# tmbdev/clstm

Hardware: AMD Instinct MI355X
Metric: text-line images/sec (fwd+bwd+CTC), 100-unit BiLSTM H=48 T~200 (higher is better)
Workload: dtype f32 (operand-exact split): forward, recurrences, CTC, decode in f32 arithmetic; the backward weight-gradient / softmax-backward products take their f32 operands split EXACTLY into three bf16 terms each (x1 + x2 + x3 = x) and sum the six bf16-MFMA products of weight >= 2^-16 in f32 -- what is dropped

## Files before the change

clstm_amd/csrc/dbgopt.h:

```cpp
#pragma once
#include <cstdlib>
#include <cstring>
#include <map>
#include <stdexcept>
#include <string>

namespace clstm {
struct DbgOptDef { const char* name; int dflt; };
inline constexpr DbgOptDef DBG_OPTS[] = {
    {"gemm_stag", 2},
    {"bwd_c32", 1},
    {"rec_x3", 1},
    {"pack_tiles", 1},
    {"fuse_wx", 1},
    {"gemm_b16mc", 1},
    {"dw_x3", 1},
    {"gemm_x3", 1},
    {"split_terms", 3},
    {"fwd_mfma", 1},
    {"bwd_mfma", 1},
    {"bwd_mfma_fused", 1},
    {"ctc_float", 0},
    {"peer_two_phase", 1},
};
inline const DbgOptDef* dbg_opt_def(const char* name) {
  for (const DbgOptDef& o : DBG_OPTS)
    if (strcmp(o.name, name) == 0) return &o;
  return nullptr;
}
inline std::map<std::string, int>& dbg_opts() {
  static std::map<std::string, int> m = [] {
    std::map<std::string, int> r;
    const char* e = getenv("CLSTM_DEBUG");
    if (e) {
      std::string s(e);
      size_t i = 0;
      while (i < s.size()) {
        size_t j = s.find(',', i);
        if (j == std::string::npos) j = s.size();
        const std::string kv = s.substr(i, j - i);
        const size_t eq = kv.find('=');
        if (!kv.empty()) {
          const std::string name = kv.substr(0, eq);
          if (eq == std::string::npos || !dbg_opt_def(name.c_str()))
            throw std::runtime_error("CLSTM_DEBUG: unknown option '" + name + "' (clstm_amd/csrc/dbgopt.h lists them as name=value)");
          r[name] = atoi(kv.c_str() + eq + 1);
        }
        i = j + 1;
      }
    }
    return r;
  }();
  return m;
}
inline int dbg_opt(const char* name) {
  const DbgOptDef* d = dbg_opt_def(name);
  if (!d) throw std::logic_error(std::string("internal: option '") + name + "' is not in DBG_OPTS");
  const auto& m = dbg_opts();
  const auto it = m.find(name);
  return it == m.end() ? d->dflt : it->second;
}
}
```

clstm_amd/csrc/gemm_dw.h:

```cpp
#pragma once
#include <type_traits>
#include "gemm_bf16.h"

namespace clstm {

struct DwSlab {
  int tile_begin, ntiles;
  int need_it;
  int dir;
  int out_z;
  int pad[3];
};

struct GemmDwArgs {
  const float* S; long long sdir; int lds; long long s_elems;
  const float* D; int M; int no4; long long d_elems;
  const int* ktab;
  int ntiles_max;
  const DwSlab* slabs;
  int nslabs;
  const int* prog;
  const int* line_off;
  int bs, prog_base, ndir;
  float* partial;
  int R, Cn;
  unsigned gx, gy;
  int* timeouts;
  int* minprog;
  int tcap;
  int* done;
  int done_target;
  long long* trace;
  int trace_base;
  const float* xS; int xlds; long long xs_elems;
  const float* xD; int xM; long long xd_elems;
  const int* xtab; const DwSlab* xslabs; int xnslabs;
  float* xpartial; int xR, xCn; unsigned xgx, xgy;
  int x3;
  int terms;
};

constexpr int DW_PF = 3;
constexpr int DW_STAB_MAX = 256;
constexpr int dw_img_floats(int nt) { return nt <= 2 ? 8192 : 2 * 2 * nt * 64 * 32 / 2; }
constexpr int dw_smem_floats(int nt) { return dw_img_floats(nt) + 2 * DW_STAB_MAX; }
static_assert(8192 >= GEMM_BT * GEMM_LDO, "epilogue tile");

constexpr int DW_WATCHDOG_POLLS = 1 << 16;

DEVFN void gemm_dw_monitor(const GemmDwArgs& a) {
  if (threadIdx.x >= 64) return;
  const int lane = threadIdx.x & 63;
  int polls = 0;
  for (;;) {
    int all = 0x3fffffff;
    int pv[2][4];
#pragma unroll
    for (int dir = 0; dir < 2; dir++)
#pragma unroll
      for (int j = 0; j < 4; j++) {
        const int b = lane + 64 * j;
        pv[dir][j] = dir < a.ndir && b < a.bs ? load_i32_wt(a.prog + ((size_t)dir * a.bs + b) * PROG_STRIDE) : 0;
      }
    for (int dir = 0; dir < a.ndir; dir++) {
      int m = 0x3fffffff;
      for (int b = lane, j = 0; b < a.bs; b += 64, j++) {
        const int T = a.line_off[b + 1] - a.line_off[b];
        const int p = (j < 4 ? pv[dir][j] : load_i32_wt(a.prog + ((size_t)dir * a.bs + b) * PROG_STRIDE)) - a.prog_base;
        const int v = p >= T ? 0x3fffffff : (p < 0 ? 0 : p);
        m = v < m ? v : m;
      }
      m = -wave_max_i(-m);
      if (lane == 0) store_i32_wt(a.minprog + dir * PROG_STRIDE, a.prog_base + (m > a.tcap ? a.tcap : m));
      all = m < all ? m : all;
    }
    if (all >= 0x3fffffff) break;
    if (++polls > (DW_WATCHDOG_POLLS << 4)) {
      if (lane == 0) {
        atomic_add_i32(a.timeouts, 1);
        for (int dir = 0; dir < a.ndir; dir++) store_i32_wt(a.minprog + dir * PROG_STRIDE, a.prog_base + a.tcap);
      }
      break;
    }
  }
}

DEVFN void gemm_dw_wait(const GemmDwArgs& a, const int dir, const int need_it) {
  const int wave = wave_uniform(threadIdx.x >> 6);
  if (wave == 0) {
    const int need = need_it < a.tcap ? need_it : a.tcap;
    const bool all = a.done && need_it >= a.tcap - 32;
    int polls = 0;
// ... 288 lines not shown
```

clstm_amd/csrc/lstm_bwd_dw.h:

```cpp
#pragma once
#include "gemm_dw.h"
#include "lstm_seq.h"

namespace clstm {

constexpr int DW_FUSED_STAB_ENTRIES = 1024;
static_assert(DW_FUSED_STAB_ENTRIES >= DW_STAB_MAX, "the items' k-tile table fits");

template <int NK4, int KU, int NT>
__global__ __launch_bounds__(64 * NK4) CLSTM_TWO_WAVES_PER_SIMD void lstm_bwd_dw_kernel(LstmSeqArgs a, GemmDwArgs g, int nrec) {
  __shared__ __attribute__((aligned(16))) float gsm[dw_img_floats(NT) + 2 * DW_FUSED_STAB_ENTRIES];
  if ((int)blockIdx.x < nrec) {
#ifndef CLSTM_HIP_EMU
    __builtin_amdgcn_s_setprio(3);
#endif
    const long long t0 = g.trace ? wall_clock() : 0;
    const int bl = (int)blockIdx.x % a.bs;
    lstm_bwd_body<NK4, KU>(a, a.order ? a.order[bl] : bl, (int)blockIdx.x / a.bs);
    if (g.done && threadIdx.x == 0) atomic_add_i32(g.done, 1);
    if (g.trace && threadIdx.x == 0) { g.trace[blockIdx.x * 4] = t0; g.trace[blockIdx.x * 4 + 2] = wall_clock(); }
  } else {
    if (threadIdx.x >= 256) return;
    gemm_dw_body<NT>(g, gsm, blockIdx.x - (unsigned)nrec);
  }
}

}
```

clstm_amd/csrc/net.inc:

```
struct Layer {
  int ni, no, nk4, nthreads;
  bool wide = false;
  int kpf = 0, kpb = 0;
  long long nwf = 0, nwb = 0;
  PackDesc pd;
  float *Wt = nullptr, *bias = nullptr, *Rf = nullptr, *Rb = nullptr, *Rwf = nullptr, *Rwb = nullptr;
  float* Wk = nullptr;
  int wk_kp = 0, wk_njp = 0;
  DevBuf<float> dCc;
  DevBuf<unsigned short> Wmf;
  DevBuf<float> mf_scale;
  DevBuf<unsigned> mf_xmax;
  long long mf_epoch = -1;
  DevBuf<unsigned short> Wmfb;
  long long mfb_epoch = -1;
  DevBuf<int> pack_tab;
  DevBuf<int> pack_inv;
  int pack_inv_state = 0;
  unsigned short *Rbf = nullptr, *Rbb = nullptr;
  DevBuf<unsigned short> R2b, D2;
  bool r2b_ready = false;
  DevBuf<unsigned short> Hb, Db;
  DevBuf<float> Rf32;
  long long* moff = nullptr;
// ... 534 lines not shown
    const int mode = dbg_opt("bwd_mfma");
    if (!mode || y.wide || bf16_gemm) return false;
    if (strict_f32 && mode < 2) return false;
    if (!(y.no == 64 || y.no == 100)) return false;
    const double lim = 2147483000.0;
    if ((double)N * ndir * 4 * y.no * 4 >= lim) return false;
    return mode >= 2 || bs >= 640;
#endif
  }
#ifndef CLSTM_HIP_EMU
  template <int NO, int NT>
  LstmMfmaBwdArgs mfma_bwd_args(Layer& y, const LstmSeqArgs& sa, hipStream_t s) {
    using Gm = MfmaBwdGeom<NO, NT>;
    if (y.mfb_epoch != params_epoch) {
      y.Wmfb.reserve((size_t)ndir * Gm::W_HALFS_PER_DIR + 64);
      MfmaBwdPackArgs p{};
      p.v = v; p.ni = y.ni; p.no = y.no; p.ntl = Gm::NTL; p.kb = Gm::KB; p.nt = NT; p.W = y.Wmfb.p;
      for (int d = 0; d < 2; d++) for (int q = 0; q < 4; q++) p.p_off[d][q] = y.pd.p_off[d][q];
      CLSTM_LAUNCH(k_pack_mfma_bwd, dim3(64, (unsigned)ndir), dim3(256), 0, s, p);
      y.mfb_epoch = params_epoch;
    }
    LstmMfmaBwdArgs a{};
    a.W = y.Wmfb.p; a.G = sa.G; a.C = sa.C; a.dH = sa.dH; a.D = sa.D; a.line_off = sa.line_off; a.order = sa.order;
    a.bs = bs; a.ndir = ndir; a.N = N; a.prog_off = sa.prog_off; a.prog_base = sa.prog_base;
    return a;
  }
  template <int NO>
  void launch_mfma_bwd_no(Layer& y, const LstmSeqArgs& sa, hipStream_t s) {
    constexpr int NT = 2;
    using Gr = MfmaBwdRowsGeom<NO, NT>;
    const LstmMfmaBwdArgs a = mfma_bwd_args<NO, NT>(y, sa, s);
    static const bool smem_set = (coop_set_smem(lstm_bwd_mfma_rows_kernel<NO, NT>, (size_t)Gr::SMEM), true);
    (void)smem_set;
    CLSTM_LAUNCH((lstm_bwd_mfma_rows_kernel<NO, NT>), dim3((unsigned)((bs + 15) / 16), (unsigned)ndir), dim3(512), (size_t)Gr::SMEM, s, a);
    g_path_count[PC_MFMA_BWD]++;
  }
  template <int NO>
  bool launch_mfma_bwd_dw_no(Layer& y, const LstmSeqArgs& sa, const GemmDwArgs& g, unsigned ngemm, hipStream_t s) {
    constexpr int NT = 2;
    using Gr = MfmaBwdRowsGeom<NO, NT>;
    const LstmMfmaBwdArgs a = mfma_bwd_args<NO, NT>(y, sa, s);
    const int ngroups = (bs + 15) / 16, nrec = ngroups * ndir;
    static const bool smem_set = (coop_set_smem(lstm_bwd_mfma_dw_kernel<NO, NT, 3>, (size_t)Gr::SMEM), true);
    (void)smem_set;
    CLSTM_LAUNCH((lstm_bwd_mfma_dw_kernel<NO, NT, 3>), dim3((unsigned)nrec + ngemm), dim3(512), (size_t)Gr::SMEM, s, a, g, nrec, ngroups);
    g_path_count[PC_MFMA_BWD]++; g_path_count[PC_MFMA_BWD_DW]++;
    return true;
  }
  bool mfma_bwd_fused_ok(const Layer& y, const GemmDwArgs& g) const {
    const int mode = dbg_opt("bwd_mfma_fused");
    return mfma_bwd_eligible(y) && mode && g.x3 && g.terms >= 3 && (mode >= 2 || bs < 900);
  }
#endif
  void launch_bwd_narrow(Layer& y, const LstmSeqArgs& a, hipStream_t s) {
#ifndef CLSTM_HIP_EMU
    if (mfma_bwd_eligible(y)) {
      if (y.no == 64) launch_mfma_bwd_no<64>(y, a, s);
      else launch_mfma_bwd_no<100>(y, a, s);
      check_launch();
      return;
    }
#endif
    launch_lstm(false, y.nk4, y.pd.ku, a, bs, y.nthreads, s);
  }
  void launch_mfma(Layer& y, bool fwd, hipStream_t s, bool save = true) {
#ifndef CLSTM_HIP_EMU
    if (save) {
      if (y.no == 64) launch_mfma_no<64, 48>(y, fwd, s);
      else if (y.no == 100) launch_mfma_no<100, 48>(y, fwd, s);
      else launch_mfma_no<128, 48>(y, fwd, s);
    } else {
      REQUIRE(mfma_nosave_ok(y), "internal: no no-save instantiation of the batched recurrence for this layer");
      if (y.no == 64) launch_mfma_no<64, 48, false>(y, fwd, s);
      else launch_mfma_no<100, 48, false>(y, fwd, s);
    }
    check_launch();
#else
    (void)y; (void)fwd; (void)s; (void)save;
#endif
  }

  void forward() {
    REQUIRE(N > 0, "set_batch first");
    RoctxRange range_("clstm:forward");
    ensure_training_buffers();
    nosave = false;
    forward_pass(true);
  }
  void forward_pass(bool save) {
    flush_line_off();
    repack();
    hipStream_t s = stream();
    if (forward_family(L[0]) == FwdFamily::Fused) { forward_fused(save); return; }
    for (int l = 0; l < (int)L.size(); l++) {
      Layer& y = L[l];
      const int M = ndir * 4 * y.no;
      const FwdFamily fam = forward_family(y);
      const bool x_from_hbf = bf16_gemm && bf16_rec && l > 0 && L[l - 1].fwd_persistent && L[l - 1].Hbf.p && y.WtbT.p && y.ni == ndir * L[l - 1].no && (y.ni & 1) == 0;
      auto run_wide = [&](LstmWideArgs w, int fx_ngx) {
        timing.begin("lstm_fwd", s);
        const WideRan ran = launch_lstm_wide(true, w, tmax, coop_sync, step_graphs, s, bf16_rec, fx_ngx);
        timing.end(s);
        if (ran == WideRan::Nothing) return false;
        y.fwd_persistent = ran == WideRan::Persistent && bf16_rec;
        y.h_f32_valid = !(y.fwd_persistent && w.skip_h);
        y.sh_valid = !(y.fwd_persistent && w.skip_s);
        if (ran == WideRan::Persistent) g_path_count[PC_FWD_PERSISTENT]++;
// ... 180 lines not shown
    h.pitems = fw_items.p; h.npitems = fw_npitems; h.gflag = fw_flags.p;
    h.W1k = W1k; h.kps = w1k_kps; h.sm_k = sm_ni; h.b1 = v + sm_off; h.Z = Z.p; h.nc = desc.nclasses;
    h.citems = fw_items.p + 4 * fw_npitems; h.ncitems = fw_ncitems;
    h.nanflag = fwd_nanflag(); h.step_no = step_no() + 1;
    h.prog = (const int*)(y.H.p + a.prog_off);
    h.nrec = bs * ndir; h.npb = fw_npitems;
    const unsigned nblk = (unsigned)(h.nrec + h.npb + fw_ncitems);
    if (save) { y.sx_valid = src0_ready; ensure_source_x(0); }
    static const char* trace_path = getenv("CLSTM_FW_TRACE");
    const size_t trace_rows = (size_t)h.nrec + fw_npitems + fw_ncitems;
    if (trace_path) { dw_trace.reserve(trace_rows * 4); HIPCHECK(hipMemsetAsync(dw_trace.p, 0, trace_rows * 4 * sizeof(long long), s)); h.trace = dw_trace.p; }
    timing.begin("lstm_fwd", s);
    REQUIRE(launch_lstm_fwd_fused(y.nk4, y.pd.ku, k, nblk, y.nthreads, s, save), "internal: no fused forward instantiation");
    timing.end(s);
    if (trace_path)
      dump_trace(trace_path, dw_trace.p, trace_rows, s,
                 "# %d recurrence rows (start - end -), %d producer items (start - done chunk), %d consumer items (start ready done ready_iteration); 100 MHz ticks\n",
                 h.nrec, fw_npitems, fw_ncitems);
  }

  bool dw_x3 = dbg_opt("dw_x3") != 0;
  int split_terms = dbg_opt("split_terms");
  bool gemm_x3_on = dbg_opt("gemm_x3") != 0;
  bool strict_f32 = false;
  bool rec_x3() const {
    if (bf16_gemm || bf16_rec || !gemm_x3_on) return false;
    return dbg_opt("rec_x3") != 0;
  }
  int clamp_split(long long want) const { return (int)std::max(1LL, std::min({want, (long long)(N + 63) / 64, 64LL})); }
  int pick_split_mc(int R, int Cn, int nbatch) const {
    const int th = gemm_mc_tile_rows(R);
    const long long tiles = (long long)((R + th - 1) / th) * ((Cn + 255) / 256) * nbatch;
    return clamp_split(device_cu_count() / tiles);
  }
  int pick_split(int R, int Cn, int nbatch = 1, int tile = GEMM_BT) const {
    const long long tiles = (long long)((R + tile - 1) / tile) * ((Cn + tile - 1) / tile) * nbatch;
    const long long target = tile == GEMM_BT ? 640 : 480;
    long long want = (target + tiles - 1) / tiles;
    if (tile == 256) want = device_cu_count() / tiles;
    return clamp_split(want);
  }

  bool overlap_eligible(const Layer& y) const {
    if (!overlap || y.wide || y.no % 16 == 0) return false;
    if (bs > PROG_LINES) return false;
    if ((overlap == 1) && (tmax < 64 || N < 2048)) return false;
    if ((double)y.D.cap * 4.0 >= 2147483000.0) return false;
    return overlap == 2 || y.nthreads >= 256;
  }
  BwdFamily backward_family(const Layer& y) const {
    if (!bf16_gemm && overlap_eligible(y)) return BwdFamily::Overlapped;
    return y.wide ? BwdFamily::Wide : BwdFamily::Narrow;
  }
  static int dw_bf16_rows(const Layer& y, int R, int Cn) { return wide_kp16_bwd(y.no) == 4 * y.no && gemm_bf16_big(R - 1, Cn) ? R - 1 : R; }
  static constexpr int DW_CHUNK = 16, DW_TAIL_PARTS = 4, DW_TAIL_CHUNKS = 2;
  void build_dw_tables() {
    if (dw_key == line_off_h && dw_nslabs > 0) return;
    std::vector<int> cb;
    for (int done = DW_CHUNK; done < tmax; done += DW_CHUNK) cb.push_back(done);
    cb.push_back(tmax);
    const int tiles_per_slab = std::min(DW_STAB_MAX, std::max(8, (int)((N / 16 + 15) / 16)));
    std::vector<std::vector<int>> tab(ndir);
    struct Sl { int tb, nt, need, dir, chunk, part; };
    std::vector<std::vector<Sl>> sl(ndir);
    for (int dir = 0; dir < ndir; dir++) {
      int cs = 0;
      for (size_t c = 0; c < cb.size(); c++) {
        const int ce = cb[c];
        const int t0 = (int)tab[dir].size() / 2;
        for (int b = 0; b < bs; b++) {
          const int off = line_off_h[b], T = line_off_h[b + 1] - off;
          if (T <= cs) continue;
          const int e = std::min(ce, T);
          const int f_lo = dir == 0 ? T - e : cs, f_hi = dir == 0 ? T - cs : e;
          for (int f = f_lo; f < f_hi; f += 16) { tab[dir].push_back(off + f); tab[dir].push_back(std::min(16, f_hi - f)); }
        }
        const int nt = (int)tab[dir].size() / 2 - t0;
        int parts = std::max(1, (nt + tiles_per_slab - 1) / tiles_per_slab);
        if (c + DW_TAIL_CHUNKS >= cb.size()) parts = std::max(parts, std::min(DW_TAIL_PARTS, std::max(1, nt / 2)));
        for (int p = 0; p < parts; p++) {
          const int a0 = t0 + (int)((long long)nt * p / parts), a1 = t0 + (int)((long long)nt * (p + 1) / parts);
          REQUIRE(a1 - a0 <= DW_STAB_MAX, "internal: weight-gradient slab longer than its LDS table");
          sl[dir].push_back(Sl{a0, a1 - a0, ce, dir, (int)c, p});
        }
        cs = ce;
      }
    }
    dw_slabs_per_dir = (int)sl[0].size();
    for (int dir = 1; dir < ndir; dir++) REQUIRE((int)sl[dir].size() == dw_slabs_per_dir, "internal: asymmetric slab lists");
    dw_ntiles_max = 0;
    for (int dir = 0; dir < ndir; dir++) dw_ntiles_max = std::max(dw_ntiles_max, (int)tab[dir].size() / 2);
    std::vector<DwSlab> slabs;
    for (int i = 0; i < dw_slabs_per_dir; i++)
      for (int dir = 0; dir < ndir; dir++) {
        const Sl& x = sl[dir][i];
        slabs.push_back(DwSlab{x.tb, x.nt, x.need, dir, dir * dw_slabs_per_dir + i, {0, 0, 0}});
      }
    dw_nslabs = (int)slabs.size();
    const size_t nk = (size_t)ndir * dw_ntiles_max * 2, nsw = slabs.size() * sizeof(DwSlab) / sizeof(int);
    dw_ktab.reserve(nk + 8);
    dw_slabs.reserve(nsw + 8);
    hipStream_t s = stream();
    int* stage = (int*)ring.acquire((nk + nsw) * sizeof(int));
    for (int dir = 0; dir < ndir; dir++) {
      std::fill(stage + (size_t)dir * dw_ntiles_max * 2, stage + (size_t)(dir + 1) * dw_ntiles_max * 2, 0);
      std::copy(tab[dir].begin(), tab[dir].end(), stage + (size_t)dir * dw_ntiles_max * 2);
    }
    memcpy(stage + nk, slabs.data(), nsw * sizeof(int));
    HIPCHECK(hipMemcpyAsync(dw_ktab.p, stage, nk * sizeof(int), hipMemcpyHostToDevice, s));
    HIPCHECK(hipMemcpyAsync(dw_slabs.p, stage + nk, nsw * sizeof(int), hipMemcpyHostToDevice, s));
    ring.commit(s);
    dw_key = line_off_h;
  }
  void backward_layer_overlapped(Layer& y, LstmSeqArgs a, int R, int Cn) {
    hipStream_t s = stream();
    build_dw_tables();
    const int M = ndir * 4 * y.no;
    const long long prog_off = (long long)y.D.cap - 64 - PROG_WORDS;
    REQUIRE(prog_off >= (long long)N * M, "internal: progress words overlap the deltas");
    prog_base += tmax + 64;
    dw_launches++;
    if (prog_base > (1 << 30)) prog_base = 1024;
    a.prog_off = prog_off;
    a.prog_base = prog_base;
    DevBuf<float>& partial = layer_partial(y);
    partial.reserve((size_t)ndir * dw_slabs_per_dir * R * Cn);
    GemmDwArgs g{};
    g.S = y.S.p; g.sdir = (long long)N * y.lds; g.lds = y.lds; g.s_elems = (long long)N * ndir * y.lds + 3;
    g.D = y.D.p; g.M = M; g.no4 = 4 * y.no; g.d_elems = (long long)N * M + 3;
    g.ktab = dw_ktab.p; g.ntiles_max = dw_ntiles_max; g.slabs = (const DwSlab*)dw_slabs.p; g.nslabs = dw_nslabs;
    g.prog = (const int*)(y.D.p + prog_off); g.line_off = line_off.p; g.bs = bs; g.prog_base = prog_base;
    g.partial = partial.p; g.R = R; g.Cn = Cn;
    g.gx = (unsigned)((Cn + GEMM_BT - 1) / GEMM_BT); g.gy = (unsigned)((R + GEMM_BT - 1) / GEMM_BT);
    g.timeouts = dev_err_words() + 1;
    if (!dw_queue.p) dw_queue.reserve(5 * PROG_STRIDE);
    g.ndir = ndir;
    g.minprog = dw_queue.p + PROG_STRIDE;
    g.tcap = tmax + 32;
    g.done = nullptr; g.done_target = 0;
    g.x3 = dw_x3;
    g.terms = split_terms;
    unsigned nextra = 0;
    if (dwx_active && &y == &L.back()) {
      const int xR = 1 + sm_ni, xCn = desc.nclasses;
      g.xS = y.srow(); g.xlds = y.ldh; g.xs_elems = (long long)N * y.ldh + 3;
      g.xD = Dz.p; g.xM = xCn; g.xd_elems = (long long)N * xCn + 3;
      g.xtab = dwx_tab.p; g.xslabs = (const DwSlab*)(dwx_tab.p + 2 * dwx_entries); g.xnslabs = dwx_nslabs;
      g.xpartial = partial_sm.p; g.xR = xR; g.xCn = xCn;
      g.xgx = (unsigned)((xCn + GEMM_BT - 1) / GEMM_BT); g.xgy = (unsigned)((xR + GEMM_BT - 1) / GEMM_BT);
      nextra = (unsigned)dwx_nslabs * g.xgx * g.xgy;
    }
    static const char* trace_path = getenv("CLSTM_DW_TRACE");
    const size_t trace_rows = (size_t)bs * ndir + (size_t)((dw_nslabs + 7) / 8) * 8 * g.gx * g.gy + 8;
    if (trace_path) { dw_trace.reserve(trace_rows * 4); g.trace = dw_trace.p; g.trace_base = bs * ndir; }
    const unsigned nblk = 1u + nextra + (unsigned)((dw_nslabs + 7) / 8) * 8u * g.gx * g.gy;
#ifndef CLSTM_HIP_EMU
    if (mfma_bwd_fused_ok(y, g)) {
      timing.begin("lstm_bwd", s);
      g.done = nullptr; g.done_target = 0;
      const bool ok = y.no == 64 ? launch_mfma_bwd_dw_no<64>(y, a, g, nblk, s) : launch_mfma_bwd_dw_no<100>(y, a, g, nblk, s);
      timing.end(s);
      check_launch();
      if (ok) return;
    }
    if (y.nthreads >= 256 && !mfma_bwd_eligible(y)) {
      timing.begin("lstm_bwd", s);
      g.done = g.minprog + 2 * PROG_STRIDE;
      dw_done_total += (unsigned)(bs * ndir);
      g.done_target = (int)dw_done_total;
      REQUIRE(launch_lstm_bwd_dw(y.nk4, y.pd.ku, a, g, bs * ndir, nblk, y.nthreads, s), "internal: no fused instantiation");
      timing.end(s);
      if (trace_path)
        dump_trace(trace_path, dw_trace.p, trace_rows, s,
                   "# rows 0..%d: recurrence workgroups (start, -, end); then one row per (slab, tile) item: start ready done need_it; 100 MHz ticks\n", bs * ndir - 1);
      return;
    }
#endif
    timing.begin("lstm_bwd", s);
    launch_bwd_narrow(y, a, s);
    timing.end(s);
    timing.begin("gemm_gates_dw", s);
    if (g.x3 && g.terms >= 3) CLSTM_LAUNCH(gemm_dw_kernel<3>, dim3(nblk), dim3(256), 0, s, g);
    else if (g.x3) CLSTM_LAUNCH(gemm_dw_kernel<2>, dim3(nblk), dim3(256), 0, s, g);
    else CLSTM_LAUNCH(gemm_dw_kernel<0>, dim3(nblk), dim3(256), 0, s, g);
    timing.end(s);
    check_launch();
  }

  void build_dwx_table() {
    if (dwx_N == N) return;
    hipStream_t s = stream();
    dwx_entries = (int)((N + 15) / 16);
    const int eps = std::min(DW_STAB_MAX, std::max(32, (dwx_entries + 63) / 64));
    dwx_nslabs = (dwx_entries + eps - 1) / eps;
    const size_t nsw = (size_t)dwx_nslabs * sizeof(DwSlab) / sizeof(int);
    dwx_tab.reserve((size_t)2 * dwx_entries + nsw + 8);
    int* stage = (int*)ring.acquire(((size_t)2 * dwx_entries + nsw) * sizeof(int));
    for (int e = 0; e < dwx_entries; e++) { stage[2 * e] = 16 * e; stage[2 * e + 1] = (int)std::min<long long>(16, N - 16LL * e); }
    DwSlab* sl = (DwSlab*)(stage + 2 * dwx_entries);
    for (int i = 0; i < dwx_nslabs; i++) sl[i] = DwSlab{eps * i, std::min(eps, dwx_entries - eps * i), 0, 0, i, {0, 0, 0}};
    for (int i = 0; i < dwx_nslabs; i++) REQUIRE(sl[i].ntiles <= DW_STAB_MAX, "internal: weight-gradient slab longer than its LDS table");
    HIPCHECK(hipMemcpyAsync(dwx_tab.p, stage, ((size_t)2 * dwx_entries + nsw) * sizeof(int), hipMemcpyHostToDevice, s));
    ring.commit(s);
    dwx_N = N;
  }
  struct ReduceTarget { bool fuse, peer; float* gdst; };
  void backward() {
    REQUIRE(N > 0, "set_batch first");
    const bool fuse = fuse_update, peer = peer_step && comm;
    fuse_update = false;
    peer_step = false; peer_pending = false;
    const ReduceTarget rt{fuse, peer, peer ? comm->peer.slot_ptr(comm->peer.seq + 1) : g};
    nbackward++;
    RoctxRange range_("clstm:backward");
    update_applied = false;
    pending_red.clear();
    deferred.armed = false;
    flush_line_off();
    repack();
    hipStream_t s = stream();
    backward_softmax();
    for (int l = (int)L.size() - 1; l >= 0; l--) {
      const BwdFamily fam = backward_family(L[l]);
      const bool bwd_persistent = backward_recurrence(l, fam);
      const BwdPlan p = backward_plan(L[l], fam, bwd_persistent);
      if (!p.dw_from_bf16) { ensure_source(l); ensure_delta_f32(l); }
      if (!backward_weight_gradient(l, p, rt)) backward_input_deltas(l, p);
    }
    if (!pending_red.empty()) {
      timing.begin("reduce_scatter", s);
      for (size_t i = 0; i < pending_red.size(); i++) reduce_layer(pending_red[i].gates, pending_red[i].extra, i + 1 == pending_red.size(), rt);
      pending_red.clear();
      timing.end(s);
      check_launch();
    }
  }
  void backward_softmax() {
    hipStream_t s = stream();
    Layer& top = L.back();
    const int nc = desc.nclasses, R = 1 + sm_ni, Cn = nc;
    const float* W1 = v + sm_off;
    const bool sm_big = bf16_gemm && gemm_x3_on && gemm_bf16_big(R, Cn) && gemm_bf16_big((int)N, sm_ni);
    int ns = sm_big ? pick_split(R, Cn, 1, GB2_BT) : pick_split(R, Cn);
    dwx_active = dw_x3 && backward_family(top) == BwdFamily::Overlapped && (long long)bs * ndir * 4 <= 3LL * device_cu_count();
    if (dwx_active) { build_dwx_table(); ns = dwx_nslabs; }
    partial_sm.reserve((size_t)ns * R * Cn);
    const GemmOperand Wk = gemm_kc(W1 + nc, nc, sm_ni, 0);
    const StorePartial wd_store{partial_sm.p, R, Cn};
    const StorePlain xd_store{top.dH.p, sm_ni};
    timing.begin("gemm_softmax_dw_dx", s);
    if (dwx_active) gemm_x3<GEMM_KC, GEMM_KC>(s, gemm_kc(Dz.p, nc, N), Wk, xd_store, (int)N, sm_ni, nc, 1, 1, split_terms);
    else if (sm_big) {
      gemm_x3_big<GEMM_MC, GEMM_MC>(s, gemm_mc(top.srow(), top.ldh, N, 32), gemm_mc(Dz.p, nc, N, 32), wd_store, R, Cn, (int)N, ns);
      gemm_x3_big<GEMM_KC, GEMM_KC>(s, gemm_kc(Dz.p, nc, N, 32), Wk, xd_store, (int)N, sm_ni, nc);
    } else {
      const GemmProblem wd = gemm_problem(gemm_mc(top.srow(), top.ldh, N), gemm_mc(Dz.p, nc, N), R, Cn, (int)N, ns);
      const GemmProblem xd = gemm_problem(gemm_kc(Dz.p, nc, N), Wk, (int)N, sm_ni, nc);
      if (gemm_x3_on) gemm_x3_pair<GEMM_MC, GEMM_MC, StorePartial, GEMM_KC, GEMM_KC, StorePlain>(s, wd, wd_store, xd, xd_store, split_terms);
      else gemm_f32_pair<GEMM_MC, GEMM_MC, StorePartial, GEMM_KC, GEMM_KC, StorePlain>(s, wd, wd_store, xd, xd_store);
    }
    timing.end(s);
    sm_red = ReduceDesc{partial_sm.p, nullptr, (long long)sm_off, ns, 1, R, Cn, nc};
    check_launch();
  }
  bool backward_recurrence(int l, BwdFamily fam) {
    Layer& y = L[l];
    hipStream_t s = stream();
    const LstmSeqArgs a = seq_args(y, false);
    if (fam == BwdFamily::Overlapped) {
      backward_layer_overlapped(y, a, 1 + y.ni + y.no, 4 * y.no);
      return false;
    }
    timing.begin("lstm_bwd", s);
    WideRan ran = WideRan::Nothing;
    int skipped_d = 0;
    if (fam == BwdFamily::Wide) {
      const LstmWideArgs w = wide_args(y, false);
      ran = launch_lstm_wide(false, w, tmax, coop_sync, step_graphs, s, bf16_rec, 0, rec_x3());
      skipped_d = w.skip_d;
    } else launch_bwd_narrow(y, a, s);
    timing.end(s);
    const bool persistent = ran == WideRan::Persistent;
    y.d_f32_valid = !(persistent && bf16_rec && skipped_d);
    if (persistent) g_path_count[PC_BWD_PERSISTENT]++;
    return persistent;
  }
  BwdPlan backward_plan(const Layer& y, BwdFamily fam, bool bwd_persistent) const {
    const int R = 1 + y.ni + y.no, Cn = 4 * y.no;
    BwdPlan p{};
    p.family = fam; p.bwd_persistent = bwd_persistent;
    p.dw_from_bf16 = bf16_gemm && bf16_rec && bwd_persistent && y.sbf_ready && y.Dbf.p && gemm_bf16_big(R, Cn);
    p.dw_rows = p.dw_from_bf16 ? dw_bf16_rows(y, R, Cn) : R;
    p.dw_bias_out = p.dw_rows < R;
    REQUIRE(!p.dw_bias_out || y.dbias.p, "internal: bias row left out of the weight-gradient product without the recurrence's per-line sums");
    p.x3_big = !bf16_gemm && y.wide && gemm_x3_on && gemm_bf16_big(R, Cn);
    p.ns = fam == BwdFamily::Overlapped ? dw_slabs_per_dir
           : p.dw_bias_out && gemm_tile256(p.dw_rows, Cn) ? pick_split_mc(p.dw_rows, Cn, ndir)
           : p.dw_from_bf16 && gemm_tile256(R, Cn) ? pick_split_mc(R, Cn, ndir)
           : (bf16_gemm || p.x3_big) && gemm_bf16_big(R, Cn) ? pick_split(R, Cn, ndir, GB2_BT) : pick_split(R, Cn, ndir);
    return p;
  }
  bool backward_weight_gradient(int l, const BwdPlan& p, const ReduceTarget& rt) {
    Layer& y = L[l];
    hipStream_t s = stream();
    const int M = ndir * 4 * y.no, R = 1 + y.ni + y.no, Cn = 4 * y.no;
    const bool product = p.family != BwdFamily::Overlapped, stacked = L.size() > 1;
    DevBuf<float>& pbuf = layer_partial(y);
    const char* const bracket = product ? "gemm_gates_dw" : stacked ? nullptr : "reduce_scatter";
    if (bracket) timing.begin(bracket, s);
    bool dx_done = false;
    if (product) {
      pbuf.reserve((size_t)ndir * p.ns * R * Cn);
      const GemmOperand src = gemm_batched(gemm_mc(y.S.p, y.lds, N), (long long)N * y.lds, ndir);
      const GemmOperand dlt = gemm_batched(gemm_mc(y.D.p, M, N, 0), 4LL * y.no, 1);
// ... 210 lines not shown
```

clstm_amd/csrc/runtime.inc:

```

static thread_local std::string g_err;
static thread_local hipStream_t g_stream = nullptr;

struct Error : std::runtime_error {
  using std::runtime_error::runtime_error;
};
#define HIPCHECK(expr)                                                                       \
  do {                                                                                       \
    hipError_t e_ = (expr);                                                                  \
    if (e_ != hipSuccess)                                                                    \
      throw Error(std::string(#expr) + " failed: " + hipGetErrorString(e_) + " (" + __FILE__ + \
                  ":" + std::to_string(__LINE__) + ")");                                     \
  } while (0)
#define REQUIRE(cond, msg)                    \
  do {                                        \
    if (!(cond)) throw Error(std::string(msg)); \
  } while (0)
#define ABI_BEGIN try {
#define ABI_END                         \
  return 0;                             \
  }                                     \
  catch (const std::exception& e) {     \
    g_err = e.what();                   \
    return 1;                           \
// ... 45 lines not shown
    cap = 0;
  }
};

struct PinnedRing {
  static const int SLOTS = 32, GROUP = 8;
  void* h[SLOTS] = {};
  size_t cap[SLOTS] = {};
  hipEvent_t ev[SLOTS / GROUP] = {};
  bool busy[SLOTS / GROUP] = {};
  int cur = SLOTS - 1;
  void* acquire(size_t bytes) {
    cur = (cur + 1) % SLOTS;
    const int g = cur / GROUP;
    if (cur % GROUP == 0 && busy[g]) { HIPCHECK(hipEventSynchronize(ev[g])); busy[g] = false; }
    if (cap[cur] < bytes) {
      if (h[cur]) (void)hipHostFree(h[cur]);
      cap[cur] = bytes * 2 + 256;
      HIPCHECK(hipHostMalloc(&h[cur], cap[cur]));
    }
    return h[cur];
  }
  void commit(hipStream_t s) {
    if (cur % GROUP != GROUP - 1) return;
    const int g = cur / GROUP;
    if (!ev[g]) HIPCHECK(hipEventCreateWithFlags(&ev[g], hipEventDisableTiming));
    HIPCHECK(hipEventRecord(ev[g], s));
    busy[g] = true;
  }
  ~PinnedRing() {
    for (int i = 0; i < SLOTS / GROUP; i++)
      if (ev[i]) (void)hipEventDestroy(ev[i]);
    for (int i = 0; i < SLOTS; i++)
      if (h[i]) (void)hipHostFree(h[i]);
  }
};

struct StoreBias {
  float* out; long long ld; const float* bias;
  DEVMFN void operator()(int r, int c, float v, int) const { out[(long long)r * ld + c] = v + bias[c]; }
  DEVMFN bool vec4() const { return (ld & 3) == 0 && (((size_t)out | (size_t)bias) & 15) == 0; }
  DEVMFN void row4(int r, int c, f32x4 v, int) const {
    const f32x4 b = *reinterpret_cast<const f32x4*>(bias + c);
    f32x4 o;
    o[0] = v[0] + b[0]; o[1] = v[1] + b[1]; o[2] = v[2] + b[2]; o[3] = v[3] + b[3];
    *reinterpret_cast<f32x4*>(out + (long long)r * ld + c) = o;
  }
};
enum PathCounter {
  PC_FWD_PERSISTENT = 0, PC_BWD_PERSISTENT = 1, PC_WX_FROM_BF16 = 2, PC_DX_FROM_BF16 = 3, PC_DW_FROM_BF16 = 4, PC_FWD_FUSED = 5,
  PC_FWD_FUSED_WX = 6, PC_PEER_EXCHANGE = 7, PC_DW_X_EXTERNAL = 8, PC_BWD_C32 = 9, PC_PACKS_FOLLOW_UPDATE = 10, PC_BWD_X3 = 11,
  PC_REPLICA_CHECK = 12, PC_DW_BIAS_OUT = 13, PC_DW_DX_ONE_LAUNCH = 14, PC_MFMA_NOSAVE = 15, PC_MFMA_FWD = 16, PC_MFMA_BWD = 17,
  PC_MFMA_BWD_DW = 18, PC_INGEST_TAIL = 19, PC_INGEST_TAIL_USED = 20, PC_MFMA_ROUTED = 21 ,
  PC_LINE_NOSAVE = 22, PC_FUSED_NOSAVE = 23, PC_PEER_TWO_PHASE = 24, PC_NORMALIZED = 25, PC_COUNT
};
static long long g_path_count[PC_COUNT];
struct StorePlain {
  float* out; long long ld;
  DEVMFN void operator()(int r, int c, float v, int) const { out[(long long)r * ld + c] = v; }
  DEVMFN bool vec4() const { return (ld & 3) == 0 && ((size_t)out & 15) == 0; }
  DEVMFN void row4(int r, int c, f32x4 v, int) const { *reinterpret_cast<f32x4*>(out + (long long)r * ld + c) = v; }
};
struct StorePartial {
  float* out; int R, Cn;
  DEVMFN void operator()(int r, int c, float v, int z) const { out[((long long)z * R + r) * Cn + c] = v; }
  DEVMFN bool vec4() const { return (Cn & 3) == 0 && ((size_t)out & 15) == 0; }
  DEVMFN void row4(int r, int c, f32x4 v, int z) const {
    *reinterpret_cast<f32x4*>(out + ((long long)z * R + r) * Cn + c) = v;
  }
};
struct StorePartialShift {
  float* out; int R, Cn;
  DEVMFN void operator()(int r, int c, float v, int z) const { out[((long long)z * R + r + 1) * Cn + c] = v; }
  DEVMFN bool vec4() const { return (Cn & 3) == 0 && ((size_t)out & 15) == 0; }
  DEVMFN void row4(int r, int c, f32x4 v, int z) const { *reinterpret_cast<f32x4*>(out + ((long long)z * R + r + 1) * Cn + c) = v; }
};
struct StorePartialRot {
  float* out; int R, Cn;
  DEVMFN void operator()(int r, int c, float v, int z) const { out[((long long)z * R + (r + 1 == R ? 0 : r + 1)) * Cn + c] = v; }
  DEVMFN bool vec4() const { return (Cn & 3) == 0 && ((size_t)out & 15) == 0; }
  DEVMFN void row4(int r, int c, f32x4 v, int z) const {
    *reinterpret_cast<f32x4*>(out + ((long long)z * R + (r + 1 == R ? 0 : r + 1)) * Cn + c) = v;
  }
};
#ifndef GEMM_BK_DW
#define GEMM_BK_DW 16
#endif
static const int kNK4Table[] = {1, 2, 4, 7, 8};
static int pick_nk4(int no) {
  int need = ((no + 3) / 4 + 3) / 4;
  for (int v : kNK4Table)
    if (v >= need) return v;
  return -1;
}
template <int NK4, int KU, bool SAVE = true>
static void launch_fwd(const LstmSeqArgs& a, int bs, int nthreads, hipStream_t s) {
  const size_t smem = (2 * 4 * (size_t)lstm_qstride(NK4) + 4) * sizeof(float);
  CLSTM_LAUNCH((lstm_fwd_kernel<NK4, KU, SAVE>), dim3(bs, a.ndir), dim3(nthreads), smem, s, a);
}
template <int NK4, int KU>
static void launch_bwd(const LstmSeqArgs& a, int bs, int nthreads, hipStream_t s) {
  const size_t smem = (2 * 16 * (size_t)lstm_qstride(NK4) + 4) * sizeof(float);
  CLSTM_LAUNCH((lstm_bwd_kernel<NK4, KU>), dim3(bs, a.ndir), dim3(nthreads), smem, s, a);
}
template <int NK4, int KU, bool SAVE = true>
static void launch_fwd_fused(const FwdFusedKernelArgs& k, unsigned nblk, int nthreads, hipStream_t s) {
  const size_t smem = (2 * 4 * (size_t)lstm_qstride(NK4) + 4) * sizeof(float);
#ifdef CLSTM_HIP_EMU
  CLSTM_LAUNCH_COOP((lstm_fwd_fused_kernel<NK4, KU, SAVE>), dim3(nblk), dim3(nthreads), smem, s, k);
#else
  CLSTM_LAUNCH((lstm_fwd_fused_kernel<NK4, KU, SAVE>), dim3(nblk), dim3(nthreads), smem, s, k);
#endif
}
static bool launch_lstm_fwd_fused(int nk4, int ku, const FwdFusedKernelArgs& k, unsigned nblk, int nthreads, hipStream_t s, bool save = true) {
#define CASE_(N, K) if (nk4 == N && ku == K) { if (save) launch_fwd_fused<N, K>(k, nblk, nthreads, s); else launch_fwd_fused<N, K, false>(k, nblk, nthreads, s); check_launch(); return true; }
  CASE_(7, 25) CASE_(7, 28) CASE_(8, 32)
#undef CASE_
  return false;
}
static int pick_ku(int no, int nk4) { return (nk4 == 7 && (no + 3) / 4 == 25) ? 25 : 4 * nk4; }
static void launch_lstm(bool fwd, int nk4, int ku, LstmSeqArgs a, int bs, int nthreads, hipStream_t s, bool save = true) {
#define CASE_(N, K) if (nk4 == N && ku == K) { \
    if (!fwd) launch_bwd<N, K>(a, bs, nthreads, s); else if (save) launch_fwd<N, K>(a, bs, nthreads, s); else launch_fwd<N, K, false>(a, bs, nthreads, s); \
    check_launch(); return; }
  CASE_(1, 4) CASE_(2, 8) CASE_(4, 16) CASE_(7, 28) CASE_(7, 25) CASE_(8, 32)
#undef CASE_
  throw Error("unsupported nhidden for the register-resident recurrence");
}

template <int NK4, int KU>
static void launch_bwd_dw(const LstmSeqArgs& a, const GemmDwArgs& g, int nrec, unsigned ngemm, int nthreads, hipStream_t s) {
  const size_t smem = (2 * 16 * (size_t)lstm_qstride(NK4) + 4) * sizeof(float);
  if (g.x3 && g.terms >= 3) CLSTM_LAUNCH((lstm_bwd_dw_kernel<NK4, KU, 3>), dim3(nrec + ngemm), dim3(nthreads), smem, s, a, g, nrec);
  else if (g.x3) CLSTM_LAUNCH((lstm_bwd_dw_kernel<NK4, KU, 2>), dim3(nrec + ngemm), dim3(nthreads), smem, s, a, g, nrec);
  else CLSTM_LAUNCH((lstm_bwd_dw_kernel<NK4, KU, 0>), dim3(nrec + ngemm), dim3(nthreads), smem, s, a, g, nrec);
}
static bool launch_lstm_bwd_dw(int nk4, int ku, const LstmSeqArgs& a, const GemmDwArgs& g, int nrec, unsigned ngemm, int nthreads, hipStream_t s) {
#define CASE_(N, K) if (nk4 == N && ku == K) { launch_bwd_dw<N, K>(a, g, nrec, ngemm, nthreads, s); check_launch(); return true; }
  CASE_(7, 25) CASE_(7, 28) CASE_(4, 16) CASE_(8, 32)
#undef CASE_
  return false;
}

static int device_cu_count() {
#ifndef CLSTM_HIP_EMU
  static int n = [] {
    int dev = 0, v = 0;
    if (hipGetDevice(&dev) != hipSuccess) return 0;
    if (hipDeviceGetAttribute(&v, hipDeviceAttributeMultiprocessorCount, dev) != hipSuccess) return 0;
    return v;
  }();
  return n;
#else
  static const int n = getenv("CLSTM_EMU_CUS") ? atoi(getenv("CLSTM_EMU_CUS")) : 16;
  return n;
#endif
}
template <class K>
static void coop_set_smem(K kernel, size_t smem) {
#ifndef CLSTM_HIP_EMU
  HIPCHECK(hipFuncSetAttribute((const void*)kernel, hipFuncAttributeMaxDynamicSharedMemorySize, (int)smem));
#endif
}
struct StepGraphCache {
  bool unsupported = false;
#ifndef CLSTM_HIP_EMU
  struct Entry { std::vector<char> key; int kind; int tmax; hipGraphExec_t exec; };
  std::vector<Entry> entries;
  hipGraphExec_t find(int kind, const std::vector<char>& key, int tmax) {
    for (auto& e : entries)
      if (e.kind == kind && e.tmax == tmax && e.key == key) return e.exec;
    return nullptr;
  }
  void put(int kind, const std::vector<char>& key, int tmax, hipGraphExec_t exec) {
    if (entries.size() >= 16) { (void)hipGraphExecDestroy(entries.front().exec); entries.erase(entries.begin()); }
    entries.push_back(Entry{key, kind, tmax, exec});
  }
  ~StepGraphCache() { for (auto& e : entries) (void)hipGraphExecDestroy(e.exec); }
#endif
};
// ... 329 lines not shown
```

Measured before the change: 226,500.

## Fuse softmax input-gradient GEMM into per-line backward recurrence prologue

Computes the softmax-layer input gradient (Dz times W) for each line inside the backward LSTM kernel, as a prologue that runs before the recurrence. It uses split-bf16 MFMA tiles staged in shared memory. This removes the separate gemm_softmax_dw_dx launch and its round trip to global memory, at the cost of extra serial work at the start of each recurrence block. The path is enabled by default through the xd_prologue option, but only for the top layer when it is not on the MFMA backward path.

```diff
diff --git a/clstm_amd/csrc/dbgopt.h b/clstm_amd/csrc/dbgopt.h
--- a/clstm_amd/csrc/dbgopt.h
+++ b/clstm_amd/csrc/dbgopt.h
@@ -17,6 +17,7 @@
     {"dw_x3", 1},
     {"gemm_x3", 1},
     {"split_terms", 3},
+    {"xd_prologue", 1},
     {"fwd_mfma", 1},
     {"bwd_mfma", 1},
     {"bwd_mfma_fused", 1},
diff --git a/clstm_amd/csrc/gemm_dw.h b/clstm_amd/csrc/gemm_dw.h
--- a/clstm_amd/csrc/gemm_dw.h
+++ b/clstm_amd/csrc/gemm_dw.h
@@ -10,6 +10,13 @@
   int dir;
   int out_z;
   int pad[3];
+};
+
+struct XdArgs {
+  GemmOperand A;
+  GemmOperand B;
+  float* out; int ld;
+  int K;
 };
 
 struct GemmDwArgs {
@@ -38,6 +45,7 @@
   float* xpartial; int xR, xCn; unsigned xgx, xgy;
   int x3;
   int terms;
+  XdArgs xd;
 };
 
 constexpr int DW_PF = 3;
diff --git a/clstm_amd/csrc/lstm_bwd_dw.h b/clstm_amd/csrc/lstm_bwd_dw.h
--- a/clstm_amd/csrc/lstm_bwd_dw.h
+++ b/clstm_amd/csrc/lstm_bwd_dw.h
@@ -1,11 +1,13 @@
 #pragma once
 #include "gemm_dw.h"
 #include "lstm_seq.h"
+#include "lstm_xd_prologue.h"
 
 namespace clstm {
 
 constexpr int DW_FUSED_STAB_ENTRIES = 1024;
 static_assert(DW_FUSED_STAB_ENTRIES >= DW_STAB_MAX, "the items' k-tile table fits");
+static_assert(xd_smem_floats(2) <= dw_img_floats(2) && xd_smem_floats(3) <= dw_img_floats(3), "the recurrence role's x.d prologue stages in the items' carve");
 
 template <int NK4, int KU, int NT>
 __global__ __launch_bounds__(64 * NK4) CLSTM_TWO_WAVES_PER_SIMD void lstm_bwd_dw_kernel(LstmSeqArgs a, GemmDwArgs g, int nrec) {
@@ -16,7 +18,11 @@
 #endif
     const long long t0 = g.trace ? wall_clock() : 0;
     const int bl = (int)blockIdx.x % a.bs;
-    lstm_bwd_body<NK4, KU>(a, a.order ? a.order[bl] : bl, (int)blockIdx.x / a.bs);
+    const int b = a.order ? a.order[bl] : bl, dir = (int)blockIdx.x / a.bs;
+    if constexpr (NT >= 2) {
+      if (g.xd.A.p) xd_prologue<NT, xd_maxu(NK4)>(gsm, g.xd, a.line_off, b, dir, a.no);
+    }
+    lstm_bwd_body<NK4, KU>(a, b, dir);
     if (g.done && threadIdx.x == 0) atomic_add_i32(g.done, 1);
     if (g.trace && threadIdx.x == 0) { g.trace[blockIdx.x * 4] = t0; g.trace[blockIdx.x * 4 + 2] = wall_clock(); }
   } else {
diff --git a/clstm_amd/csrc/lstm_xd_prologue.h b/clstm_amd/csrc/lstm_xd_prologue.h
--- /dev/null
+++ b/clstm_amd/csrc/lstm_xd_prologue.h
@@ -0,0 +1,159 @@
+#pragma once
+#include "gemm_dw.h"
+#include "lstm_seq.h"
+
+namespace clstm {
+
+constexpr int XD_KB = 3;
+constexpr int XD_MAX_K = 32 * XD_KB;
+constexpr int XD_ROWS = 32;
+constexpr int XD_UNITS = XD_ROWS * XD_KB * 4;
+constexpr int XD_RING = 3;
+constexpr int xd_maxu(int nk4) { return nk4 <= 1 ? 6 : nk4 == 2 ? 3 : nk4 <= 7 ? 2 : 1; }
+constexpr int xd_smem_floats(int nt) { return 2 * nt * XD_KB * XD_ROWS * 32 / 2; }
+
+template <int NT, int MAXU>
+DEVFN void xd_prologue(float* smem, const XdArgs& x, const int* line_off, const int b, const int dir, const int no) {
+  static_assert(NT == 2 || NT == 3, "two or three bf16 terms per operand");
+  unsigned short* img = reinterpret_cast<unsigned short*>(smem);
+  const int tid = threadIdx.x, lane = tid & 63, wave = wave_uniform(tid >> 6);
+  const int nthreads = blockDim.x;
+  const int off = line_off[b];
+  const int T = line_off[b + 1] - off;
+  if (T <= 0) return;
+  const int K = x.K;
+  const BufF32 abuf = make_buf(x.A.p + (size_t)off * x.A.ld, (size_t)(x.A.elems - (long long)off * x.A.ld) * 4);
+  const BufF32 bbuf = make_buf(x.B.p, (size_t)x.B.elems * 4);
+  const BufF32 obuf = make_buf(x.out + (size_t)off * x.ld, (size_t)T * x.ld * 4);
+  const int fk = lane >> 4, fi = lane & 15;
+  constexpr int IMG = XD_ROWS * 32;
+  constexpr int BUFH = NT * XD_KB * IMG;
+
+  auto load_round = [&](const int r, f32x4 (&ra)[MAXU][2]) {
+#pragma unroll
+    for (int i = 0; i < MAXU; i++) {
+      if (i * nthreads + (tid & ~63) >= XD_UNITS) break;
+      const int u = i * nthreads + tid;
+      const int row = r * XD_ROWS + u / (XD_KB * 4), ku = u % (XD_KB * 4);
+      const unsigned o = u < XD_UNITS && row < T ? ((unsigned)row * (unsigned)x.A.ld + (unsigned)((ku >> 2) * 32 + (ku & 3) * 8)) * 4u : BUF_OOB_BASE;
+      ra[i][0] = buf_load4(abuf, o);
+      ra[i][1] = buf_load4(abuf, o + 16u);
+    }
+  };
+  auto stage_round = [&](unsigned short* dst, const f32x4 (&ra)[MAXU][2]) {
+#pragma unroll
+    for (int i = 0; i < MAXU; i++) {
+      if (i * nthreads + (tid & ~63) >= XD_UNITS) break;
+      const int u = i * nthreads + tid;
+      if (u < XD_UNITS) {
+        const int row = u / (XD_KB * 4), ku = u % (XD_KB * 4), kb = ku >> 2, kk = (ku & 3) * 8;
+        float v[8];
+#pragma unroll
+        for (int e = 0; e < 8; e++) v[e] = kb * 32 + kk + e < K ? ra[i][e >> 2][e & 3] : 0.0f;
+        const int o = kb * IMG + row * 32 + (((kk >> 3) ^ gb2_sw(row)) << 3);
+#pragma unroll
+        for (int t = 0; t < NT; t++) {
+          const u16x8 h = bf16_pack8(v);
+          *reinterpret_cast<u16x8*>(dst + t * XD_KB * IMG + o) = h;
+          if (t + 1 < NT) {
+#pragma unroll
+            for (int e = 0; e < 8; e++) v[e] -= __builtin_bit_cast(float, (unsigned)h[e] << 16);
+          }
+        }
+      }
+    }
+  };
+
+  f32x4 ring[XD_RING][MAXU][2];
+#pragma unroll
+  for (int p = 0; p < XD_RING; p++) {
+    load_round(p, ring[p]);
+    SCHED_FENCE();
+  }
+
+  const int n = wave * 16 + fi;
+  const bool has_tile = wave * 16 < no;
+  u16x8 bt[XD_KB][NT];
+  if (has_tile) {
+    const unsigned brow = n < no ? (unsigned)(dir * no + n) * (unsigned)x.B.ld * 4u : BUF_OOB_BASE;
+    f32x4 rb[XD_KB][2];
+#pragma unroll
+    for (int kb = 0; kb < XD_KB; kb++) {
+      rb[kb][0] = buf_load4(bbuf, brow + (unsigned)(kb * 32 + fk * 8) * 4u);
+      rb[kb][1] = buf_load4(bbuf, brow + (unsigned)(kb * 32 + fk * 8 + 4) * 4u);
+    }
+#pragma unroll
+    for (int kb = 0; kb < XD_KB; kb++) {
+      float v[8];
+#pragma unroll
+      for (int i = 0; i < 8; i++) v[i] = kb * 32 + fk * 8 + i < K ? rb[kb][i >> 2][i & 3] : 0.0f;
+#pragma unroll
+      for (int t = 0; t < NT; t++) {
+        const u16x8 h = bf16_pack8(v);
+        bt[kb][t] = h;
+        if (t + 1 < NT) {
+#pragma unroll
+          for (int i = 0; i < 8; i++) v[i] -= __builtin_bit_cast(float, (unsigned)h[i] << 16);
+        }
+      }
+    }
+  }
+
+  const int nrounds = (T + XD_ROWS - 1) / XD_ROWS;
+  const int fofs = fi * 32 + ((fk ^ gb2_sw(fi)) << 3);
+  const unsigned ocol = n < no ? (unsigned)(dir * no + n) * 4u : BUF_OOB_BASE;
+  auto round = [&](const int r, f32x4 (&ra)[MAXU][2]) {
+    unsigned short* cur = img + (r & 1) * BUFH;
+    stage_round(cur, ra);
+    wait_lgkmcnt0();
+    wg_barrier();
+    COMPILER_MEMORY_BARRIER();
+    load_round(r + XD_RING, ra);
+    SCHED_FENCE();
+    if (has_tile) {
+      f32x4 acc[2];
+#pragma unroll
+      for (int m = 0; m < 2; m++)
+#pragma unroll
+        for (int q = 0; q < 4; q++) acc[m][q] = 0.0f;
+#pragma unroll
+      for (int kb = 0; kb < XD_KB; kb++) {
+        u16x8 at[NT][2];
+#pragma unroll
+        for (int t = 0; t < NT; t++)
+#pragma unroll
+          for (int m = 0; m < 2; m++) at[t][m] = *reinterpret_cast<const u16x8*>(cur + (t * XD_KB + kb) * IMG + m * 16 * 32 + fofs);
+#pragma unroll
+        for (int w = NT - 1; w >= 0; w--)
+#pragma unroll
+          for (int ta = w; ta >= 0; ta--)
+#pragma unroll
+            for (int m = 0; m < 2; m++) acc[m] = mfma16x16x32_bf16(at[ta][m], bt[kb][w - ta], acc[m]);
+      }
+#pragma unroll
+      for (int m = 0; m < 2; m++)
+#pragma unroll
+        for (int q = 0; q < 4; q++) {
+          const int row = r * XD_ROWS + m * 16 + fk * 4 + q;
+          buf_store(obuf, row < T ? (unsigned)row * (unsigned)x.ld * 4u + ocol : BUF_OOB_BASE, acc[m][q]);
+        }
+    }
+  };
+  for (int r = 0; r < nrounds; r += XD_RING) {
+#pragma unroll
+    for (int p = 0; p < XD_RING; p++)
+      if (r + p < nrounds) round(r + p, ring[p]);
+  }
+  drain_vmem();
+  __syncthreads();
+}
+
+template <int NK4, int KU, int NT>
+__global__ __launch_bounds__(64 * NK4) CLSTM_TWO_WAVES_PER_SIMD void lstm_bwd_xd_kernel(LstmSeqArgs a, XdArgs x) {
+  __shared__ __attribute__((aligned(16))) float xsm[xd_smem_floats(NT)];
+  const int b = a.order ? a.order[blockIdx.x] : (int)blockIdx.x;
+  xd_prologue<NT, xd_maxu(NK4)>(xsm, x, a.line_off, b, (int)blockIdx.y, a.no);
+  lstm_bwd_body<NK4, KU>(a, b, (int)blockIdx.y);
+}
+
+}
diff --git a/clstm_amd/csrc/net.inc b/clstm_amd/csrc/net.inc
--- a/clstm_amd/csrc/net.inc
+++ b/clstm_amd/csrc/net.inc
@@ -610,7 +610,11 @@
     return mfma_bwd_eligible(y) && mode && g.x3 && g.terms >= 3 && (mode >= 2 || bs < 900);
   }
 #endif
-  void launch_bwd_narrow(Layer& y, const LstmSeqArgs& a, hipStream_t s) {
+  void launch_bwd_narrow(Layer& y, const LstmSeqArgs& a, hipStream_t s, const XdArgs* xd = nullptr) {
+    if (xd) {
+      REQUIRE(launch_lstm_bwd_xd(y.nk4, y.pd.ku, a, *xd, split_terms, bs, y.nthreads, s), "internal: no per-line backward instantiation");
+      return;
+    }
 #ifndef CLSTM_HIP_EMU
     if (mfma_bwd_eligible(y)) {
       if (y.no == 64) launch_mfma_bwd_no<64>(y, a, s);
@@ -897,6 +901,17 @@
     if (!bf16_gemm && overlap_eligible(y)) return BwdFamily::Overlapped;
     return y.wide ? BwdFamily::Wide : BwdFamily::Narrow;
   }
+  bool xd_in_launch() const {
+    const Layer& top = L.back();
+    return dwx_active && !mfma_bwd_eligible(top) && desc.nclasses <= XD_MAX_K && top.nthreads >= 64 * ((top.no + 15) / 16) &&
+           top.nthreads * xd_maxu(top.nk4) >= XD_UNITS &&
+           dbg_opt("xd_prologue") != 0;
+  }
+  XdArgs xd_args() const {
+    const Layer& top = L.back();
+    const int nc = desc.nclasses;
+    return XdArgs{gemm_kc(Dz.p, nc, N), gemm_kc(v + sm_off + nc, nc, sm_ni, 0), top.dH.p, sm_ni, nc};
+  }
   static int dw_bf16_rows(const Layer& y, int R, int Cn) { return wide_kp16_bwd(y.no) == 4 * y.no && gemm_bf16_big(R - 1, Cn) ? R - 1 : R; }
   static constexpr int DW_CHUNK = 16, DW_TAIL_PARTS = 4, DW_TAIL_CHUNKS = 2;
   void build_dw_tables() {
@@ -986,6 +1001,8 @@
     g.x3 = dw_x3;
     g.terms = split_terms;
     unsigned nextra = 0;
+    const bool xd = &y == &L.back() && xd_in_launch();
+    if (xd) { g.xd = xd_args(); g_path_count[PC_XD_PROLOGUE]++; }
     if (dwx_active && &y == &L.back()) {
       const int xR = 1 + sm_ni, xCn = desc.nclasses;
       g.xS = y.srow(); g.xlds = y.ldh; g.xs_elems = (long long)N * y.ldh + 3;
@@ -1022,7 +1039,7 @@
     }
 #endif
     timing.begin("lstm_bwd", s);
-    launch_bwd_narrow(y, a, s);
+    launch_bwd_narrow(y, a, s, xd ? &g.xd : nullptr);
     timing.end(s);
     timing.begin("gemm_gates_dw", s);
     if (g.x3 && g.terms >= 3) CLSTM_LAUNCH(gemm_dw_kernel<3>, dim3(nblk), dim3(256), 0, s, g);
@@ -1093,9 +1110,11 @@
     const GemmOperand Wk = gemm_kc(W1 + nc, nc, sm_ni, 0);
     const StorePartial wd_store{partial_sm.p, R, Cn};
     const StorePlain xd_store{top.dH.p, sm_ni};
-    timing.begin("gemm_softmax_dw_dx", s);
-    if (dwx_active) gemm_x3<GEMM_KC, GEMM_KC>(s, gemm_kc(Dz.p, nc, N), Wk, xd_store, (int)N, sm_ni, nc, 1, 1, split_terms);
-    else if (sm_big) {
+    const bool launches = !xd_in_launch();
+    if (launches) timing.begin("gemm_softmax_dw_dx", s);
+    if (dwx_active) {
+      if (launches) gemm_x3<GEMM_KC, GEMM_KC>(s, gemm_kc(Dz.p, nc, N), Wk, xd_store, (int)N, sm_ni, nc, 1, 1, split_terms);
+    } else if (sm_big) {
       gemm_x3_big<GEMM_MC, GEMM_MC>(s, gemm_mc(top.srow(), top.ldh, N, 32), gemm_mc(Dz.p, nc, N, 32), wd_store, R, Cn, (int)N, ns);
       gemm_x3_big<GEMM_KC, GEMM_KC>(s, gemm_kc(Dz.p, nc, N, 32), Wk, xd_store, (int)N, sm_ni, nc);
     } else {
@@ -1104,7 +1123,7 @@
       if (gemm_x3_on) gemm_x3_pair<GEMM_MC, GEMM_MC, StorePartial, GEMM_KC, GEMM_KC, StorePlain>(s, wd, wd_store, xd, xd_store, split_terms);
       else gemm_f32_pair<GEMM_MC, GEMM_MC, StorePartial, GEMM_KC, GEMM_KC, StorePlain>(s, wd, wd_store, xd, xd_store);
     }
-    timing.end(s);
+    if (launches) timing.end(s);
     sm_red = ReduceDesc{partial_sm.p, nullptr, (long long)sm_off, ns, 1, R, Cn, nc};
     check_launch();
   }
diff --git a/clstm_amd/csrc/runtime.inc b/clstm_amd/csrc/runtime.inc
--- a/clstm_amd/csrc/runtime.inc
+++ b/clstm_amd/csrc/runtime.inc
@@ -121,7 +121,7 @@
   PC_FWD_FUSED_WX = 6, PC_PEER_EXCHANGE = 7, PC_DW_X_EXTERNAL = 8, PC_BWD_C32 = 9, PC_PACKS_FOLLOW_UPDATE = 10, PC_BWD_X3 = 11,
   PC_REPLICA_CHECK = 12, PC_DW_BIAS_OUT = 13, PC_DW_DX_ONE_LAUNCH = 14, PC_MFMA_NOSAVE = 15, PC_MFMA_FWD = 16, PC_MFMA_BWD = 17,
   PC_MFMA_BWD_DW = 18, PC_INGEST_TAIL = 19, PC_INGEST_TAIL_USED = 20, PC_MFMA_ROUTED = 21 ,
-  PC_LINE_NOSAVE = 22, PC_FUSED_NOSAVE = 23, PC_PEER_TWO_PHASE = 24, PC_NORMALIZED = 25, PC_COUNT
+  PC_LINE_NOSAVE = 22, PC_FUSED_NOSAVE = 23, PC_PEER_TWO_PHASE = 24, PC_NORMALIZED = 25, PC_XD_PROLOGUE = 26, PC_COUNT
 };
 static long long g_path_count[PC_COUNT];
 struct StorePlain {
@@ -195,6 +195,17 @@
   CASE_(1, 4) CASE_(2, 8) CASE_(4, 16) CASE_(7, 28) CASE_(7, 25) CASE_(8, 32)
 #undef CASE_
   throw Error("unsupported nhidden for the register-resident recurrence");
+}
+
+static bool launch_lstm_bwd_xd(int nk4, int ku, const LstmSeqArgs& a, const XdArgs& x, int terms, int bs, int nthreads, hipStream_t s) {
+#define CASE_(N, K) if (nk4 == N && ku == K) { \
+    const size_t smem = (2 * 16 * (size_t)lstm_qstride(N) + 4) * sizeof(float); \
+    if (terms >= 3) CLSTM_LAUNCH((lstm_bwd_xd_kernel<N, K, 3>), dim3(bs, a.ndir), dim3(nthreads), smem, s, a, x); \
+    else CLSTM_LAUNCH((lstm_bwd_xd_kernel<N, K, 2>), dim3(bs, a.ndir), dim3(nthreads), smem, s, a, x); \
+    check_launch(); return true; }
+  CASE_(1, 4) CASE_(2, 8) CASE_(4, 16) CASE_(7, 28) CASE_(7, 25) CASE_(8, 32)
+#undef CASE_
+  return false;
 }
 
 template <int NK4, int KU>
```

New measurement: 229,800 (median of 6 runs). 1.5% higher.
